# Victarry/Image-Generation-models

Hardware: AMD Instinct MI355X
Metric: ddpm_cifar10_32x32_train_images_per_sec (higher is better)
Workload: dtype bf16; 1 GPU; DDPM CIFAR-10 32x32, UNet 128/1-2-4, T=1000 (BASELINE configs[1]): train step B=128/GPU + hipGraph denoise step B=64; per_gpu_batch=128, global_batch=128, parallelism=dp1, step_launch=hipGraph replay, denoise_batch=64, rccl_ranks=1, state_finite=True, matmul=bf16 MFMA, fp32 accumulate

## Files before the change

image-generation-models_amd/csrc/conv_pw.hip:

```cpp
#include "tr_common.h"

#ifndef MI_PW_PABL
#define MI_PW_PABL 0
#endif
#ifndef MI_PW_GNSABL
#define MI_PW_GNSABL 0
#endif
#ifndef MI_PW_FXABL
#define MI_PW_FXABL 0
#endif
#ifdef MI_PW_TIMING
__device__ uint32_t g_pw_ts[1024 * 4 * 5 * 64];
__device__ __forceinline__ uint32_t pw_wlane(uint32_t val, uint32_t lane, uint32_t v) {
    uint32_t keep;
    asm volatile("s_mov_b32 %1, m0\n\ts_mov_b32 m0, %3\n\ts_nop 0\n\tv_writelane_b32 %0, %2, m0\n\ts_mov_b32 m0, %1"
                 : "+v"(v), "=&s"(keep) : "s"(__builtin_amdgcn_readfirstlane(val)), "s"(__builtin_amdgcn_readfirstlane(lane)));
    return v;
}
extern "C" int mi_debug_pw_ts(uint32_t* host_out) { return (int)hipMemcpyFromSymbol(host_out, HIP_SYMBOL(g_pw_ts), sizeof(g_pw_ts)); }
#endif

namespace {

typedef uint32_t u32x2 __attribute__((ext_vector_type(2)));
// ... 1 lines not shown
__device__ __attribute__((aligned(16))) uint32_t g_zero_page3[64];

struct PwArgs {
    const uint16_t* x; const uint16_t* x2; const uint16_t* w; const float* bias; const float* res; void* y;
    int N, H, W, K, Nc, K1, ldx, ldx2, ldy, ldr, accumulate, flip;
    int TH, TI, XP, tiles_per_img, xmap;
    int qmap, gx, gy;
    uint32_t tpi_magic, cpq_magic, nch_magic, cpg_magic; int ppx, cpq, lnsub;
    const void* zero;
    float* gsum;
    const float* coef;
    const float* sums; const float* gamma; const float* beta; const float* temb;
    int ldt, cpg, hw, ng; float eps;
    double icnt;
    int ksplit; float* sk_part; int* sk_flag;
};

constexpr int pw_xp(int pt) { return pt == 256 ? 320 : pt == 128 ? 192 : 128; }

__device__ __forceinline__ int pw_fastdiv(int x, uint32_t magic) { return magic ? (int)__umulhi((uint32_t)x, magic) : x; }
inline uint32_t pw_magic(int d) { return d > 1 ? (uint32_t)((0x100000000ULL + (unsigned)d - 1) / (unsigned)d) : 0u; }

__device__ __forceinline__ void glds16s(const void* sbase, uint32_t voff, uint32_t lds_dst) {
    const uint64_t p = (uint64_t)(uintptr_t)sbase;
    const uint32_t lo = __builtin_amdgcn_readfirstlane((uint32_t)p), hi = __builtin_amdgcn_readfirstlane((uint32_t)(p >> 32));
    const uint64_t q = ((uint64_t)hi << 32) | lo;
    const uint32_t dst = __builtin_amdgcn_readfirstlane(lds_dst);
    uint32_t keep;
    asm volatile("s_mov_b32 %0, m0\n\ts_mov_b32 m0, %3\n\ts_nop 0\n\tglobal_load_lds_dwordx4 %1, %2\n\ts_mov_b32 m0, %0"
                 : "=&s"(keep) : "v"(voff), "s"(q), "s"(dst) : "memory");
// ... 51 lines not shown
    constexpr bool TIMED = VAR == 0 && !IN32 && !F32;
    uint32_t tv[5] = {0u, 0u, 0u, 0u, 0u};
    uint64_t tprev = 0;
    if constexpr (TIMED) {
        tprev = __builtin_amdgcn_s_memtime();
        tv[4] = pw_wlane((uint32_t)wall_clock64(), 7, tv[4]);
        tv[4] = pw_wlane((uint32_t)tprev, 3, tv[4]);
    }
#define MI_PW_STAMP(SET, LANE) do { if constexpr (TIMED) { tv[SET] = pw_wlane((uint32_t)tprev, (LANE), tv[SET]); tprev = __builtin_amdgcn_s_memtime(); } } while (0)
#define MI_PW_NOW(LANE) do { if constexpr (TIMED) { tv[4] = pw_wlane((uint32_t)__builtin_amdgcn_s_memtime(), (LANE), tv[4]); } } while (0)
#else
#define MI_PW_STAMP(SET, LANE) do {} while (0)
#define MI_PW_NOW(LANE) do {} while (0)
#endif
    static_assert(PT != 256 || (VAR < 2 && !IN32 && !F32), "256-pixel tiles: the plain bf16 conv (with or without the GroupNorm sums)");
    constexpr bool FUSE = VAR >= 2, GNS = VAR == 1;
    static_assert(!F32 || (VAR == 0 && !IN32 && !OUT16), "exact-fp32 mode: the plain conv, fp32 in and out");
    constexpr int PCK = F32 ? 32 : 64;
    constexpr int ESZ = F32 ? 4 : 2, EPP = 16 / ESZ;
    constexpr int BH = PT / 32;
    constexpr int PXBUF = pw_xp(PT) * 128;
    constexpr int PXPW = pw_xp(PT) / 8 / 4;
    extern __shared__ __attribute__((aligned(16))) uint8_t lds_raw[];
    const uint32_t lds0 = (uint32_t)(uintptr_t)lds_raw;
    const int t = threadIdx.x, l = t & 63;
    const int wv = __builtin_amdgcn_readfirstlane(t >> 6);
    int bx = blockIdx.x;
    if (a.xmap) {
        const int xcd = bx & 7, slot = bx >> 3, q = pw_fastdiv(slot, a.tpi_magic);
        bx = (xcd + 8 * q) * a.tiles_per_img + (slot - q * a.tiles_per_img);
    }
// ... 29 lines not shown
        constexpr int ks0 = decltype(ksc)::value, over = ks0 >= 4 ? 1 : 0, ks = ks0 - 4 * over, part = decltype(partc)::value;
        constexpr int t0 = (9 * part + NPART - 1) / NPART, t1 = (9 * (part + 1) + NPART - 1) / NPART;
        const uint32_t voff = wl16 + (uint32_t)cof(ch + over) * 4096;
        static_for<t0, t1>([&](auto tc) {
            constexpr int tp = decltype(tc)::value;
            gload16s<ks * 1024>(WB[ks & 1][tp], wtap[tp], voff);
        });
    };

    auto load_w1 = [&](int ch, auto ksc, auto tapc) {
        constexpr int ks0 = decltype(ksc)::value, over = ks0 >= 4 ? 1 : 0, ks = ks0 - 4 * over, tp = decltype(tapc)::value;
        const uint32_t voff = wl16 + (uint32_t)cof(ch + over) * 4096;
        gload16s<ks * 1024>(WB[ks & 1][tp], wtap[tp], voff);
    };

    constexpr bool EARLYW = VAR < 2 && !IN32;
    if constexpr (EARLYW) {
        MI_PW_NOW(10);
        static_for<0, NPART>([&](auto pc) { load_w3(0, std::integral_constant<int, 0>{}, pc); });
        __builtin_amdgcn_sched_barrier(0);
    }


    int xpix[PXPW];
    const bool w8 = a.W == 8;
    const int xcol = ((l & 7) ^ (w8 ? (((l >> 4) & 3) | (((wv >> 1) & 1) << 2)) : ((4 * wv + (l >> 4)) & 7))) * EPP;
    int img0;
    {
        int y0;
        if (a.TI > 1) { img0 = bx * a.TI; y0 = 0; }
        else { img0 = pw_fastdiv(bx, a.tpi_magic); y0 = (bx - img0 * a.tiles_per_img) * a.TH; }
// ... 650 lines not shown
        __builtin_amdgcn_s_barrier();
        asm volatile("" ::: "memory");
        if (t < 32) {
            const int q = t >> 2, k = t & 3;
            const float v = red[(0 * 8 + q) * 4 + k] + red[(1 * 8 + q) * 4 + k] + red[(2 * 8 + q) * 4 + k] + red[(3 * 8 + q) * 4 + k];
            const int slab = (n0 >> 4) + q;
            if (slab * 16 < a.Nc) {
                const int img = a.TI > 1 ? img0 + (k >> 1) : img0;
                gsum_add(a.gsum, ((size_t)img * (a.Nc >> 4) + slab) * 2 + (k & 1), v);
            }
        }
        };
    __builtin_amdgcn_s_barrier();
    asm volatile("" ::: "memory");
    MI_PW_NOW(13);
    const bool tile16 = OUT16 && !a.res && !a.accumulate;
    if (tile16) {
        if constexpr (OUT16) {
            typedef __attribute__((address_space(3))) u32x2 lds_u32x2;
            typedef __attribute__((address_space(3))) u32x4 lds_u32x4e;
            if (live) {
#pragma unroll
                for (int rq = 0; rq < 4; ++rq) {
                    const int ck = 8 * wv + 2 * rq + (l >> 5);
                    typedef __attribute__((address_space(3))) f32x4 lds_f32x4b;
                    const f32x4 bq = *(lds_f32x4b*)(uintptr_t)(lds0 + BIASL + 16 * ck);
#pragma unroll
                    for (int i = 0; i < BH; ++i) {
                        const int p = ep_p0 + i * a.W;
                        *(lds_u32x2*)(uintptr_t)(lds0 + p * 256 + ((ck ^ ((p & 15) << 1)) << 3)) =
                            u32x2{pack_bf16(acc[i][4 * rq] + bq.x, acc[i][4 * rq + 1] + bq.y), pack_bf16(acc[i][4 * rq + 2] + bq.z, acc[i][4 * rq + 3] + bq.w)};
                    }
                }
            }
            __syncthreads();
            MI_PW_NOW(14);
            const int j = t & 15, col = n0 + 8 * j;
            float gs[2][2] = {{0.f, 0.f}, {0.f, 0.f}};
            if (col < a.Nc) {
#pragma unroll
                for (int it = 0; it < PT / 16; ++it) {
                    const int p = it * 16 + (t >> 4);
                    const u32x4 o = *(lds_u32x4e*)(uintptr_t)(lds0 + p * 256 + (((2 * j) ^ ((p & 15) << 1)) << 3));
                    *reinterpret_cast<u32x4*>(reinterpret_cast<uint16_t*>(a.y) + ((size_t)m0 + p) * a.ldy + col) = o;
                    if constexpr (GNS && MI_PW_GNSABL != 2) {
#pragma unroll
                        for (int q = 0; q < 4; ++q) {
                            const float e0 = __uint_as_float(o[q] << 16), e1 = __uint_as_float(o[q] & 0xffff0000u);
                            gs[PT >= 256 ? 0 : it >> 2][0] += e0 + e1; gs[PT >= 256 ? 0 : it >> 2][1] += e0 * e0 + e1 * e1;
                        }
                    }
// ... 820 lines not shown
        if (d->K % 128 || d->K1 % 128 || d->K1 <= 0 || d->K1 > d->K || d->Nc % 64 || d->ldx % 4 || (d->K1 != d->K && d->ldx2 % 4)) return false;
        return ((long)d->N * d->OH * d->OW) % 128 == 0;
    }
    if (f32) {
        if (d->KH != 1 || d->KW != 1 || d->pad != 0 || d->stride != 1 || d->mode != 0 || d->IH != d->OH || d->IW != d->OW) return false;
        if (d->K % 64 || d->K1 % 64 || d->K1 <= 0 || d->K1 > d->K || d->Nc % 64 || d->ldx % 4 || (d->K1 != d->K && d->ldx2 % 4)) return false;
        return ((long)d->N * d->OH * d->OW) % 128 == 0;
    }
    if (d->KH != 1 || d->KW != 1 || d->pad != 0 || d->stride != 1 || d->mode != 1) return false;
    if (d->IH != d->OH || d->IW != d->OW) return false;
    if (d->K % 128 || d->K1 % 128 || d->K1 <= 0 || d->K1 > d->K || d->Nc % 64 || d->ldx % 8 || (d->K1 != d->K && d->ldx2 % 8)) return false;
    return ((long)d->N * d->OH * d->OW) % 128 == 0;
}

struct PwGn { const float* sums; const float* gamma; const float* beta; const float* temb; int ldt, G; float eps; };

static int pw_launch(const char* who, const MiConvDesc* d, const void* x, const void* x2, const void* w_frag_bf16, const float* bias,
                     const float* residual, void* y, int out_bf16, int var, float* gsum, const float* coef, void* stream,
                     const PwGn* gn = nullptr, bool in32 = false, bool f32 = false) {
    PwArgs a{};
    if (!d || !x || !w_frag_bf16 || !y) return mi_set_error(-1, "%s: null argument", who);
    const int pt = pw_pick_tile(d, var, &a.TH, &a.TI, in32, f32, &a.ksplit);
    if (!pt) return mi_set_error(-1, "%s: descriptor not supported by the private-weight-stream conv kernel", who);
    int dev_ = 0;
    (void)hipGetDevice(&dev_);
    if (a.ksplit > 1) {
        uint8_t* ws = reinterpret_cast<uint8_t*>(g_pw_sk_ws[dev_ & 63].load(std::memory_order_acquire));
        a.sk_flag = reinterpret_cast<int*>(ws); a.sk_part = reinterpret_cast<float*>(ws + PW_SK_FLAG_BYTES);
#ifdef MI_PW_SK_ABL
        a.sk_flag = nullptr;
#endif
    }
    if (d->K1 != d->K && !x2) return mi_set_error(-1, "%s: two-source split without x2", who);
    if ((((uintptr_t)x | (uintptr_t)(x2 ? x2 : x) | (uintptr_t)w_frag_bf16) & 15) != 0) return mi_set_error(-1, "%s: operands must be 16-byte aligned", who);
    if (d->ldy % 8 || (residual && d->ldr % 4)) return mi_set_error(-1, "%s: output pixel stride must be a multiple of 8, the residual's of 4", who);
    if (var >= 2 && (a.TI != 1 || d->K1 != d->K))
        return mi_set_error(-1, "%s: the fused variants need one image per tile and one source", who);
    if (var == 2 && (!coef || ((uintptr_t)coef & 15)))
        return mi_set_error(-1, "%s: the fused variant needs a 16-byte aligned coefficient tensor", who);
    if (var == 3) {
        if (!gn || !gn->sums || !gn->gamma || !gn->beta || gn->G <= 0 || d->K % gn->G || (d->K / gn->G) % 16 || d->K / gn->G > 64)
            return mi_set_error(-1, "%s: sums, gamma, beta; K / G in {16, 32, 64}", who);
        if ((((uintptr_t)gn->gamma | (uintptr_t)gn->beta | (uintptr_t)gn->sums) & 7) || ((uintptr_t)gn->sums & 15) || (gn->temb && (((uintptr_t)gn->temb & 15) || gn->ldt % 4)))
            return mi_set_error(-1, "%s: misaligned GroupNorm operands", who);
        a.sums = gn->sums; a.gamma = gn->gamma; a.beta = gn->beta; a.temb = gn->temb; a.ldt = gn->ldt; a.cpg = d->K / gn->G;
        a.cpg_magic = pw_magic(a.cpg); a.ng = gn->G; a.hw = d->OH * d->OW; a.eps = gn->eps; a.icnt = 1.0 / (MI_GSUM_SCALE * (double)a.hw * (double)a.cpg);
    }
    if (var == 1 && (!gsum || d->Nc % 16)) return mi_set_error(-1, "%s: GroupNorm sums need Nc %% 16 == 0 and a sum buffer", who);
    a.x = (const uint16_t*)x; a.x2 = (const uint16_t*)(x2 ? x2 : x); a.w = (const uint16_t*)w_frag_bf16; a.bias = bias; a.res = residual; a.y = y;
    a.N = d->N; a.H = d->OH; a.W = d->OW; a.K = d->K; a.Nc = d->Nc; a.K1 = d->K1; a.ldx = d->ldx; a.ldx2 = x2 ? d->ldx2 : d->ldx;
    a.ldy = d->ldy; a.ldr = d->ldr; a.accumulate = d->accumulate; a.flip = d->transposed ? 1 : 0;
    a.gsum = gsum; a.coef = coef;
    a.tiles_per_img = a.TI > 1 ? 1 : a.H / a.TH;
    a.XP = a.TI * (a.TH + 2) * a.W;
    a.xmap = a.TI == 1 && a.tiles_per_img > 1 && a.N % 8 == 0;
    static std::atomic<const void*> zero_pages[64];
    const void* zero_page = zero_pages[dev_ & 63].load(std::memory_order_acquire);
    if (!zero_page) {
        void* p_ = nullptr;
        if (hipGetSymbolAddress(&p_, HIP_SYMBOL(g_zero_page3)) != hipSuccess || !p_) return mi_set_error(-1, "%s: zero page address", who);
        zero_pages[dev_ & 63].store(p_, std::memory_order_release);
        zero_page = p_;
    }
// ... 29 lines not shown
    } else if (in32) {
        if (pt == 64) switch (var) {
            case 1: if (out_bf16) MI_PW_GO_X(true, 1, 64); else MI_PW_GO_X(false, 1, 64); break;
            case 2: if (out_bf16) MI_PW_GO_X(true, 2, 64); else MI_PW_GO_X(false, 2, 64); break;
            case 3: if (out_bf16) MI_PW_GO_X(true, 3, 64); else MI_PW_GO_X(false, 3, 64); break;
            default: if (out_bf16) MI_PW_GO_X(true, 0, 64); else MI_PW_GO_X(false, 0, 64); break;
        } else switch (var) {
            case 1: if (out_bf16) MI_PW_GO_X(true, 1, 128); else MI_PW_GO_X(false, 1, 128); break;
            case 2: if (out_bf16) MI_PW_GO_X(true, 2, 128); else MI_PW_GO_X(false, 2, 128); break;
            case 3: if (out_bf16) MI_PW_GO_X(true, 3, 128); else MI_PW_GO_X(false, 3, 128); break;
            default: if (out_bf16) MI_PW_GO_X(true, 0, 128); else MI_PW_GO_X(false, 0, 128); break;
        }
    } else if (pt == 256) switch (var) {
        case 1: if (out_bf16) MI_PW_GO_T(true, 1, 256); else MI_PW_GO_T(false, 1, 256); break;
        default: if (out_bf16) MI_PW_GO_T(true, 0, 256); else MI_PW_GO_T(false, 0, 256); break;
    } else if (pt == 64) switch (var) {
        case 1: if (out_bf16) MI_PW_GO_T(true, 1, 64); else MI_PW_GO_T(false, 1, 64); break;
        case 2: if (out_bf16) MI_PW_GO_T(true, 2, 64); else MI_PW_GO_T(false, 2, 64); break;
        case 3: if (out_bf16) MI_PW_GO_T(true, 3, 64); else MI_PW_GO_T(false, 3, 64); break;
        default: if (out_bf16) MI_PW_GO_T(true, 0, 64); else MI_PW_GO_T(false, 0, 64); break;
    } else switch (var) {
        case 1: if (out_bf16) MI_PW_GO_T(true, 1, 128); else MI_PW_GO_T(false, 1, 128); break;
        case 2: if (out_bf16) MI_PW_GO_T(true, 2, 128); else MI_PW_GO_T(false, 2, 128); break;
        case 3: if (out_bf16) MI_PW_GO_T(true, 3, 128); else MI_PW_GO_T(false, 3, 128); break;
        default: if (out_bf16) MI_PW_GO_T(true, 0, 128); else MI_PW_GO_T(false, 0, 128); break;
    }
#undef MI_PW_GO_T
#undef MI_PW_GO_X
    hipError_t e_ = hipGetLastError();
    return e_ == hipSuccess ? 0 : mi_set_error((int)e_, "%s: %s", who, hipGetErrorString(e_));
// ... 43 lines not shown
    return (d && pw_pick_tile(d, 2, &th, &ti) && ti == 1 && d->K1 == d->K) ? 1 : 0;
}
extern "C" int mi_conv3x3_pw_gn_mish_tile(const MiConvDesc* d) {
    int th, ti;
    const int pt = d ? pw_pick_tile(d, 2, &th, &ti) : 0;
    return (pt && ti == 1 && d->K1 == d->K) ? pt : 0;
}

extern "C" int mi_conv3x3_pw(const MiConvDesc* d, const void* x, const void* x2, const void* w_frag_bf16, const float* bias,
                             const float* residual, void* y, int out_bf16, void* stream) {
    return pw_launch(__func__, d, x, x2, w_frag_bf16, bias, residual, y, out_bf16, 0, nullptr, nullptr, stream);
}
extern "C" int mi_conv3x3_pw_gnsums(const MiConvDesc* d, const void* x, const void* x2, const void* w_frag_bf16, const float* bias,
                                    const float* residual, void* y, int out_bf16, float* gsum, void* stream) {
    return pw_launch(__func__, d, x, x2, w_frag_bf16, bias, residual, y, out_bf16, 1, gsum, nullptr, stream);
}
extern "C" int mi_conv3x3_pw_x32_supported(const MiConvDesc* d) {
    int th, ti;
    return (d && pw_pick_tile(d, 0, &th, &ti, true)) ? 1 : 0;
}
extern "C" int mi_conv3x3_pw_x32_tile(const MiConvDesc* d) {
    int th, ti;
    return d ? pw_pick_tile(d, 0, &th, &ti, true) : 0;
}
extern "C" int mi_conv3x3_pw_x32(const MiConvDesc* d, const float* x, const float* x2, const void* w_frag_bf16, const float* bias,
                                 const float* residual, void* y, int out_bf16, float* gsum, void* stream) {
    return pw_launch(__func__, d, x, x2, w_frag_bf16, bias, residual, y, out_bf16, gsum ? 1 : 0, gsum, nullptr, stream, nullptr, true);
}
extern "C" int mi_conv3x3_pw_f32_tile(const MiConvDesc* d) {
    int th, ti;
// ... 341 lines not shown
```

image-generation-models_amd/src/models/ddpm.py:

```python
from __future__ import annotations

import math
import os
from functools import partial
from typing import Dict, List, Optional, Sequence, Tuple

import numpy as np
import torch
from torch import nn

from ..ops import functional as K
from .base import BaseModel, ValidationResult

_HEADS, _DHEAD = 4, 32
_GN_GROUPS = 8


def _mode_id(name: str) -> int:
    if name not in ("fp32", "bf16"):
        raise ValueError(f"compute mode must be 'fp32' or 'bf16', got {name!r}")
    return K.MODE_BF16 if name == "bf16" else K.MODE_FP32


class _Entry:
# ... 183 lines not shown
            raise ValueError("dim must be a multiple of 8")
        self.channels = channels
        self.dim = dim
        self.with_time_emb = bool(with_time_emb)
        arch = _Arch(dim, tuple(dim_mults), channels, out_dim, with_time_emb)
        object.__setattr__(self, "_arch", arch)
        self.compute_mode = os.environ.get("MI_DDPM_MODE", "fp32")
        self.block_storage = os.environ.get("MI_DDPM_STORAGE", "bf16")
        self.fuse_gn_conv = os.environ.get("MI_DDPM_FUSE_GN", "auto")
        self.s2_wgrad_tr = K.debug_knob("MI_DDPM_S2_TR", "1") != "0"
        self.final_block16 = K.debug_knob("MI_DDPM_FINAL16", "1") != "0"
        self.ends16 = K.debug_knob("MI_DDPM_ENDS16", "1") != "0"
        self.dual_out = K.debug_knob("MI_DDPM_DUAL_OUT", "1") != "0"
        self.fuse_ln_qkv = K.debug_knob("MI_DDPM_FUSE_LN", "1") != "0"
        self.fuse_ln_qkv_train = K.debug_knob("MI_DDPM_FUSE_LN_TRAIN", "1") != "0"
        self.small_cin_dual = K.debug_knob("MI_DDPM_CIN_DUAL", "1") != "0"
        self.cin_dual_chores = K.debug_knob("MI_DDPM_CIN_CHORES", "1") != "0"
        self.fold_attn = K.debug_knob("MI_DDPM_FOLD_ATTN", "0") == "1"
        self.small_cout_bwd1 = K.debug_knob("MI_DDPM_COUT_BWD1", "1") != "0"
        self.fuse_final = K.debug_knob("MI_DDPM_FUSE_FINAL", "1") != "0"
        self.accumulate_grads = False
        self.grad_ready_hook = None

        flat = torch.zeros(arch.flat_numel)
        for e in arch.entries:
            if e.init == "kaiming":
                w = torch.empty(e.shape)
                nn.init.kaiming_uniform_(w, a=math.sqrt(5))
                e.logical_view(flat).copy_(w)
            elif e.init == "ubias":
# ... 295 lines not shown
                ok2 = K.fast3x3_supported(B, inp.shape[1], inp.shape[2], co, co)
                lo16 = ok2[0] and ok2[1] and not (auto and K.conv3x3_uses_splitk(B, inp.shape[1], inp.shape[2], co, co))
            k1 = inp.shape[3] if x2 is not None else None
            c1_16 = (lo16 and ci % 32 == 0 and all(K.fast3x3_supported(B, inp.shape[1], inp.shape[2], ci, co, k1))
                     and not (auto and K.conv3x3_uses_splitk(B, inp.shape[1], inp.shape[2], ci, co, k1)))
            if (not c1_16 and lo16 and self.ends16 and x2 is None and K.small_cin_supported(3, ci, co, wgrad=True)
                    and K.small_cin_bf16_supported(3, B, inp.shape[1], inp.shape[2], ci, co, K.ld_of(inp))):
                c1_16 = True
            inp_c, x2_c = inp, x2
            if c1_16 and use_sh and inp.dtype == torch.float32 and inp.shape[3] % 8 == 0:
                inp_c, x2_c = shadow(inp), (shadow(x2) if x2 is not None else None)
            elif c1_16 and eval16 and x2 is None and id(inp) in sh:
                inp_c = sh[id(inp)][1]
            tb = tb_all[:, blk["tcol"]:blk["tcol"] + co] if tb_all is not None else None
            hw = inp.shape[1] * inp.shape[2]
            fmode = str(self.fuse_gn_conv)
            sums_ok = ((co // _GN_GROUPS) % 16 == 0 and hw % 32 == 0 and ci % 32 == 0
                       and all(K.fast3x3_supported(B, inp.shape[1], inp.shape[2], ci, co, k1)))
            fuse = (not record and mode == K.MODE_BF16 and fmode != "0" and c1_16 == lo16
                    and K.conv3x3_gn_mish_supported(B, inp.shape[1], inp.shape[2], co, co))
            if fuse and fmode == "auto":
                fuse = lo16 and sums_ok and K.conv3x3_pw_gn_mish_picked(B, inp.shape[1], inp.shape[2], co, co)
            sums = None
            if fuse and fmode in ("2", "auto") and sums_ok:
                sums = take_sums(co, inp.device)
            r_pre = None
            if (blk["res"] and x2 is None and sums is None and self.small_cin_dual and K.small_cin_supported(3, ci, co)
                    and K.small_cin_dual_supported(B, inp.shape[1], inp.shape[2], ci, co, K.ld_of(inp))):
                od = BF if (c1_16 and K.small_cin_bf16_supported(3, B, inp.shape[1], inp.shape[2], ci, co, K.ld_of(inp))) else torch.float32
                if not record and mode == K.MODE_BF16 and zpool[0] is None and str(self.fuse_gn_conv) != "0" and self.cin_dual_chores:
                    zpool[0] = torch.empty(2 * B * (sum(rb["cout"] // 16 + 1 for rb in A.res_blocks) + A.dim // 16 + 1), device=inp.device, dtype=torch.int64)
                    zfill = zpool[0]
                else:
                    zfill = None
                c1, r_pre = K.conv_small_cin_fwd_dual(inp, sv[pre + "block1.block.0.weight"], sv[pre + "block1.block.0.bias"],
                                                      sv[pre + "res_conv.weight"], sv[pre + "res_conv.bias"], co, out_dtype=od, zero=zfill,
                                                      gather=tb_pending.pop() if tb_pending else None)
            else:
                c1 = conv(inp_c, pre + "block1.block.0.", 3, 1, 1, x2=x2_c, out_dtype=BF if c1_16 else torch.float32, gn_sums=sums)
            c2 = None
            if fuse:
                if sums is not None:
                    st1 = None
                    c2 = K.conv3x3_gn_mish(c1, None, wf_sh[offs[pre + "block2.block.0.weight"]:], K=co, Nc=co, bias=sv[pre + "block2.block.0.bias"],
                                           gn=(sums, sv[pre + "block1.block.1.weight"], sv[pre + "block1.block.1.bias"], tb, _GN_GROUPS, 1e-5),
                                           wq=wfq_sh[offs[pre + "block2.block.0.weight"]:])
                else:
                    st1, coef = K.gn_stats_coef(c1, sv[pre + "block1.block.1.weight"], sv[pre + "block1.block.1.bias"], temb=tb)
                    c2 = K.conv3x3_gn_mish(c1, coef, wf_sh[offs[pre + "block2.block.0.weight"]:], K=co, Nc=co, bias=sv[pre + "block2.block.0.bias"],
                                           wq=wfq_sh[offs[pre + "block2.block.0.weight"]:])
                h1 = None
            if c2 is None:
                h1, st1 = K.gn_mish_fwd(c1, sv[pre + "block1.block.1.weight"], sv[pre + "block1.block.1.bias"], temb=tb,
                                        out_dtype=BF if lo16 else torch.float32)
                c2 = conv(h1, pre + "block2.block.0.", 3, 1, 1, out_dtype=BF if lo16 else torch.float32)
            r = inp
            if r_pre is not None:
                r = r_pre
            elif blk["res"]:
                r = None
                if inp_c is not inp and inp_c.dtype == BF and (x2 is None or x2_c is not None):
                    r = conv(inp_c, pre + "res_conv.", 1, x2=x2_c, soft=True)
                if r is None:
                    r = conv(inp, pre + "res_conv.", 1, x2=x2)
            if want_out16 and (use_sh or (eval16 and out16_in_eval)) and co % 32 == 0:
                out, st2, out16 = K.gn_mish_fwd(c2, sv[pre + "block2.block.1.weight"], sv[pre + "block2.block.1.bias"], residual=r, want16=True)
                sh[id(out)] = (out, out16)
            else:
                out, st2 = K.gn_mish_fwd(c2, sv[pre + "block2.block.1.weight"], sv[pre + "block2.block.1.bias"], residual=r)
            if record:
                tape.append(("res", blk, inp, x2, c1, st1, h1, c2, st2, out, inp_c, x2_c))
            return out

        def attention(at, inp, feeds_s2=False):
            pre = at["pre"]
            c = inp.shape[3]
            a16 = (mode == K.MODE_BF16 and self.block_storage in ("bf16", "auto") and B % 8 == 0
                   and all(K.fast1x1_supported(B, inp.shape[1], inp.shape[2], c, 3 * _HEADS * _DHEAD))
                   and all(K.fast1x1_supported(B, inp.shape[1], inp.shape[2], _HEADS * _DHEAD, c)))
            dt = BF if a16 else torch.float32
            nq = 3 * _HEADS * _DHEAD
            if (a16 and self.fuse_ln_qkv and (not record or self.fuse_ln_qkv_train) and inp.dtype == torch.float32
                    and K.ln_conv1x1_supported(B, inp.shape[1], inp.shape[2], c, nq, K.ld_of(inp))):
# ... 564 lines not shown
```

image-generation-models_amd/src/ops/functional.py:

```python
from __future__ import annotations

import ctypes as C
import functools
import os
from typing import Optional, Tuple

import torch

from .lib import ROWSUM_MAX, MiConvDesc, MiGnDesc, MiRowSum, MiWgradDesc, check, load_library

MODE_FP32, MODE_BF16 = 0, 1


def debug_knob(name: str, default: str) -> str:
    if os.environ.get("MI_DEBUG_KNOBS") == "1":
        return os.environ.get(name, default)
    return default
PROBE = None


CONV_AUTO = os.environ.get("MI_CONV_AUTO", "1") == "1"


USE_CONV_PW = CONV_AUTO and debug_knob("MI_CONV_PW", "1") == "1"
# ... 314 lines not shown
              "mi_conv3x3_bf16w_io")
    else:
        check(lib.mi_conv3x3_bf16w(C.byref(d), _p(x), _p(x2), _p(wsh), _p(bias), _p(residual), _p(out), _stream()),
              "mi_conv3x3_bf16w")
    if e0 is not None:
        bm, ck, sk = C.c_int(), C.c_int(), C.c_int()
        lib.mi_conv3x3_bf16w_tile(C.byref(d), io, C.byref(bm), C.byref(ck), C.byref(sk))
        nb = (N * H * W * K * _esz(x) + N * H * W * Nc * (_esz(out) * (2 if accumulate else 1) + _esz(residual))
              + ksize * ksize * K * Nc * 2)
        _probe_close(e0, f"conv3x3_halo_kernel<{bm.value}, {ck.value}, {ksize}, {'true' if sk.value else 'false'}, {io}, {8 if bm.value == 256 or (bm.value == 128 and ck.value == 64) else 4}>",
                     2.0 * N * H * W * Nc * K * ksize * ksize,
                     f"N{N} {H}x{W} K{K}{'(2src)' if x2 is not None else ''}->{Nc} flip{int(flip)} acc{int(accumulate)} io{io}", nb)
    return (out, y16) if want16 else out


def gn_stats_coef(x, gamma, beta, *, groups=8, eps=1e-5, temb=None):
    _need_gpu(x)
    N, H, W, Cc = x.shape
    stats = torch.empty((N, groups, 2), device=x.device, dtype=torch.float32)
    coef = torch.empty((3, N, Cc), device=x.device, dtype=torch.float32)
    d = MiGnDesc(N=N, HW=H * W, C=Cc, G=groups, eps=eps, ldx=ld_of(x), ldy=Cc, ldr=0)
    e0 = _probe_open()
    check(load_library().mi_gn_stats_coef(C.byref(d), _p(x), _p(gamma), _p(beta), _p(temb), ld_of(temb) if temb is not None else 0,
                                          _p(stats), _p(coef), _b16(x), _stream()), "mi_gn_stats_coef")
    if e0 is not None:
        _probe_close(e0, f"gn_mish_fwd_kernel<io{_b16(x)}> (statistics only)", 0.0, f"N{N} HW{H * W} C{Cc}", N * H * W * Cc * _esz(x))
    return stats, coef


GSUM_SCALE = float(1 << 20)
# ... 1409 lines not shown
```

image-generation-models_amd/src/ops/lib.py:

```python
from __future__ import annotations

import ctypes as C
import os

_PKG_ROOT = os.path.dirname(os.path.dirname(os.path.dirname(os.path.abspath(__file__))))
_LIB = None


def library_path() -> str:
    return os.environ.get("MI_DDPM_LIB", os.path.join(_PKG_ROOT, "lib", "libmi_ddpm.so"))


class MiConvDesc(C.Structure):
    _fields_ = [(n, C.c_int) for n in (
        "N", "IH", "IW", "OH", "OW", "K", "Nc", "KH", "KW", "stride", "pad", "transposed", "w_kn", "mode",
        "K1", "ldx", "ldx2", "ldy", "ldr", "accumulate")]


class MiWgradDesc(C.Structure):
    _fields_ = [(n, C.c_int) for n in (
        "N", "GH", "GW", "DH", "DW", "Ci", "Cj", "KH", "KW", "stride", "pad", "gather_i", "mode", "I1",
        "ldp", "ldp2", "ldq")]


# ... 78 lines not shown
    "mi_debug_conv_pw_splitk": [_I],
    "mi_ln_conv1x1_pw_supported": [C.POINTER(MiConvDesc)],
    "mi_ln_conv1x1_pw": [C.POINTER(MiConvDesc), _P, _P, _P, C.c_float, _P, _P, _P, _P],
    "mi_ln_conv1x1_pw_dual": [C.POINTER(MiConvDesc), _P, _P, _P, C.c_float, _P, _P, _P, _P, _I, _P],
    "mi_conv1x1_pw_f32_supported": [C.POINTER(MiConvDesc)],
    "mi_conv1x1_pw_f32": [C.POINTER(MiConvDesc), _P, _P, _P, _P, _P, _P, _P],
    "mi_pack_weights_f32frag": [_I, _P, _I, _P, _P, _P, _P],
    "mi_conv3x3_pw_x32_supported": [C.POINTER(MiConvDesc)],
    "mi_conv3x3_pw_x32_tile": [C.POINTER(MiConvDesc)],
    "mi_conv3x3_pw_x32": [C.POINTER(MiConvDesc), _P, _P, _P, _P, _P, _P, _I, _P, _P],
    "mi_conv3x3_pw": [C.POINTER(MiConvDesc), _P, _P, _P, _P, _P, _P, _I, _P],
    "mi_conv3x3_pw_gn_mish_supported": [C.POINTER(MiConvDesc)],
    "mi_conv1x1_pw_supported": [C.POINTER(MiConvDesc)],
    "mi_conv1x1_pw": [C.POINTER(MiConvDesc), _P, _P, _P, _P, _P, _P, _I, _P, _I, _P],
    "mi_conv3x3_pw_gnsums": [C.POINTER(MiConvDesc), _P, _P, _P, _P, _P, _P, _I, _P, _P],
    "mi_conv3x3_pw_gn_mish": [C.POINTER(MiConvDesc), _P, _P, _P, _P, _P, _I, _P],
    "mi_conv3x3_pw_gn_mish_sums": [C.POINTER(MiConvDesc), _P, _P, _P, _P, _P, _I, _I, _F, _P, _P, _P, _I, _P],
    "mi_conv3x3_pw_x32_gn_mish_supported": [C.POINTER(MiConvDesc)],
    "mi_conv3x3_pw_x32_gn_mish_tile": [C.POINTER(MiConvDesc)],
    "mi_conv3x3_pw_gn_mish_tile": [C.POINTER(MiConvDesc)],
    "mi_conv3x3_pw_x32_gn_mish": [C.POINTER(MiConvDesc), _P, _P, _P, _P, _P, _I, _P],
    "mi_conv3x3_pw_x32_gn_mish_sums": [C.POINTER(MiConvDesc), _P, _P, _P, _P, _P, _I, _I, _F, _P, _P, _P, _I, _P],
    "mi_gn_stats_coef": [C.POINTER(MiGnDesc), _P, _P, _P, _P, _I, _P, _P, _I, _P],
    "mi_conv3x3_gn_mish_supported": [C.POINTER(MiConvDesc)],
    "mi_conv3x3_gn_mish_tile": [C.POINTER(MiConvDesc), C.POINTER(C.c_int), C.POINTER(C.c_int)],
    "mi_conv3x3_gn_mish": [C.POINTER(MiConvDesc), _P, _P, _P, _P, _P, _I, _P],
    "mi_conv3x3_small_cin_fwd": [_I, _I, _I, _I, _I, _P, _I, _P, _P, _P, _I, _P],
    "mi_conv3x3_small_cin_wgrad": [_I, _I, _I, _I, _I, _P, _I, _P, _I, _P, _P],
    "mi_conv1x1_small_cout": [_I, _I, _I, _I, _P, _I, _P, _I, _P, _P, _P, _I, _I, _P],
    "mi_conv1x1_small_cout_ws": [_I, _I, _I, _I, _P, _I, _P, _I, _P, _P, _P, _I, _I, _P, _Z, _P],
# ... 150 lines not shown
```

include/mi_ddpm.h:

```cpp
#ifndef MI_DDPM_H
#define MI_DDPM_H
#include <stddef.h>
#include <stdint.h>

#ifdef __cplusplus
extern "C" {
#endif

#define MI_ABI_VERSION 4
#define MI_MODE_FP32 0
#define MI_MODE_BF16 1

int mi_abi_version(void);
const char* mi_last_error(void);

typedef struct MiConvDesc {
    int N;
    int IH, IW;
    int OH, OW;
    int K;
    int Nc;
    int KH, KW, stride, pad;
    int transposed;
    int w_kn;
// ... 63 lines not shown
int mi_ln_conv1x1_pw_dual(const MiConvDesc* d, const float* x, const float* ln_g, const float* ln_b, float eps, const void* w_frag_bf16,
                          const float* bias, void* y_bf16, void* ln_bf16, int ldl, void* stream);
int mi_conv1x1_pw_f32_supported(const MiConvDesc* d);
int mi_conv1x1_pw_f32(const MiConvDesc* d, const float* x, const float* x2, const float* w_frag_f32, const float* bias,
                      const float* residual, float* y, void* stream);
int mi_pack_weights_f32frag(int nent, const void* entries_dev, int total_tiles, const float* master, float* wdq32, float* wfq32,
                            void* stream);
int mi_debug_conv_pw_tile(int pt);
int mi_debug_conv_pw_auto256(int min_workgroups);
int mi_debug_conv1x1_pw_nloop(int on);
int mi_conv3x3_pw_tile(const MiConvDesc* d);
int mi_conv3x3_pw(const MiConvDesc* d, const void* x, const void* x2, const void* w_frag_bf16, const float* bias,
                  const float* residual, void* y, int out_bf16, void* stream);
int mi_conv3x3_pw_gnsums(const MiConvDesc* d, const void* x, const void* x2, const void* w_frag_bf16, const float* bias,
                         const float* residual, void* y, int out_bf16, float* gsum, void* stream);
int mi_conv3x3_pw_gn_mish_supported(const MiConvDesc* d);
int mi_conv3x3_pw_gn_mish_tile(const MiConvDesc* d);
int mi_conv3x3_pw_gn_mish(const MiConvDesc* d, const void* x, const float* coef, const void* w_frag_bf16, const float* bias,
                          void* y, int out_bf16, void* stream);
int mi_conv3x3_pw_gn_mish_sums(const MiConvDesc* d, const void* x, const float* sums, const float* gamma, const float* beta,
                               const float* temb, int ldt, int G, float eps, const void* w_frag_bf16, const float* bias,
                               void* y, int out_bf16, void* stream);
int mi_conv3x3_pw_x32_gn_mish_supported(const MiConvDesc* d);
int mi_conv3x3_pw_x32_gn_mish_tile(const MiConvDesc* d);
int mi_conv3x3_pw_x32_gn_mish(const MiConvDesc* d, const float* x, const float* coef, const void* w_frag_bf16, const float* bias,
                              void* y, int out_bf16, void* stream);
int mi_conv3x3_pw_x32_gn_mish_sums(const MiConvDesc* d, const float* x, const float* sums, const float* gamma, const float* beta,
                                   const float* temb, int ldt, int G, float eps, const void* w_frag_bf16, const float* bias,
                                   void* y, int out_bf16, void* stream);
int mi_conv1x1_pw_supported(const MiConvDesc* d);
// ... 296 lines not shown
```

Before: 26180 images/s.

## Fold GroupNorm+Mish into 3x3 conv epilogue for 8x8 resblocks

Adds conv kernel variants that compute GroupNorm statistics, the affine, Mish, the time-embedding add and optionally the residual add inside the conv epilogue, for 8x8 images where one tile covers whole images. The aim is to drop separate gn_mish_fwd launches and the extra re-reads of the conv output in the training forward pass. This costs more epilogue work and LDS reductions per tile, and it only applies to 8x8 layers, so the number of layers affected is small.

```diff
diff --git a/image-generation-models_amd/csrc/conv_pw.hip b/image-generation-models_amd/csrc/conv_pw.hip
--- a/image-generation-models_amd/csrc/conv_pw.hip
+++ b/image-generation-models_amd/csrc/conv_pw.hip
@@ -39,6 +39,7 @@
     int ldt, cpg, hw, ng; float eps;
     double icnt;
     int ksplit; float* sk_part; int* sk_flag;
+    void* y2; float* stats; const float* gres; uint16_t* y16; int ldy2, ldgr, ldy16;
 };
 
 constexpr int pw_xp(int pt) { return pt == 256 ? 320 : pt == 128 ? 192 : 128; }
@@ -120,7 +121,9 @@
 #define MI_PW_NOW(LANE) do {} while (0)
 #endif
     static_assert(PT != 256 || (VAR < 2 && !IN32 && !F32), "256-pixel tiles: the plain bf16 conv (with or without the GroupNorm sums)");
-    constexpr bool FUSE = VAR >= 2, GNS = VAR == 1;
+    constexpr bool FUSE = VAR == 2 || VAR == 3, GNS = VAR == 1;
+    constexpr bool GNF = VAR == 4 || VAR == 5;
+    static_assert(!GNF || (OUT16 && !IN32 && !F32 && (PT == 64 || PT == 128)), "GroupNorm fold: bf16 conv output, 64- or 128-pixel tiles");
     static_assert(!F32 || (VAR == 0 && !IN32 && !OUT16), "exact-fp32 mode: the plain conv, fp32 in and out");
     constexpr int PCK = F32 ? 32 : 64;
     constexpr int ESZ = F32 ? 4 : 2, EPP = 16 / ESZ;
@@ -180,7 +183,7 @@
         gload16s<ks * 1024>(WB[ks & 1][tp], wtap[tp], voff);
     };
 
-    constexpr bool EARLYW = VAR < 2 && !IN32;
+    constexpr bool EARLYW = (VAR < 2 || GNF) && !IN32;
     if constexpr (EARLYW) {
         MI_PW_NOW(10);
         static_for<0, NPART>([&](auto pc) { load_w3(0, std::integral_constant<int, 0>{}, pc); });
@@ -861,7 +864,7 @@
     __builtin_amdgcn_s_barrier();
     asm volatile("" ::: "memory");
     MI_PW_NOW(13);
-    const bool tile16 = OUT16 && !a.res && !a.accumulate;
+    const bool tile16 = GNF || (OUT16 && !a.res && !a.accumulate);
     if (tile16) {
         if constexpr (OUT16) {
             typedef __attribute__((address_space(3))) u32x2 lds_u32x2;
@@ -882,6 +885,122 @@
             }
             __syncthreads();
             MI_PW_NOW(14);
+            if constexpr (GNF) {
+                constexpr int NI = PT / 64, NR = PT / 16;
+                const int j = t & 15, pr = t >> 4, col = n0 + 8 * j;
+                const f32x4 gq0 = *reinterpret_cast<const f32x4*>(a.gamma + col), gq1 = *reinterpret_cast<const f32x4*>(a.gamma + col + 4);
+                const f32x4 bq0 = *reinterpret_cast<const f32x4*>(a.beta + col), bq1 = *reinterpret_cast<const f32x4*>(a.beta + col + 4);
+                f32x4 tq[NI][2];
+#pragma unroll
+                for (int im = 0; im < NI; ++im) {
+                    tq[im][0] = tq[im][1] = f32x4{0.f, 0.f, 0.f, 0.f};
+                    if (a.temb) {
+                        const float* tp = a.temb + (size_t)(img0 + im) * a.ldt + col;
+                        tq[im][0] = *reinterpret_cast<const f32x4*>(tp); tq[im][1] = *reinterpret_cast<const f32x4*>(tp + 4);
+                    }
+                }
+                f32x4 rq[VAR == 5 ? NR : 1][2];
+                if constexpr (VAR == 5) {
+#pragma unroll
+                    for (int it = 0; it < NR; ++it) {
+                        const float* rp = a.gres + ((size_t)m0 + it * 16 + pr) * a.ldgr + col;
+                        rq[it][0] = *reinterpret_cast<const f32x4*>(rp); rq[it][1] = *reinterpret_cast<const f32x4*>(rp + 4);
+                    }
+                }
+                u32x4 o[NR];
+#pragma unroll
+                for (int it = 0; it < NR; ++it) {
+                    const int p = it * 16 + pr;
+                    o[it] = *(lds_u32x4e*)(uintptr_t)(lds0 + p * 256 + (((2 * j) ^ ((p & 15) << 1)) << 3));
+                    *reinterpret_cast<u32x4*>(reinterpret_cast<uint16_t*>(a.y) + ((size_t)m0 + p) * a.ldy + col) = o[it];
+                }
+                auto gn_sum = [&](float (&v)[NI], float* red) {
+#pragma unroll
+                    for (int im = 0; im < NI; ++im) {
+                        v[im] += __shfl_xor(v[im], 1, 64);
+                        if (a.cpg >= 32) v[im] += __shfl_xor(v[im], 2, 64);
+                        if (a.cpg >= 64) v[im] += __shfl_xor(v[im], 4, 64);
+                        v[im] += __shfl_xor(v[im], 16, 64); v[im] += __shfl_xor(v[im], 32, 64);
+                    }
+                    if (l < 16) {
+#pragma unroll
+                        for (int im = 0; im < NI; ++im) red[(wv * 16 + l) * NI + im] = v[im];
+                    }
+                    asm volatile("s_waitcnt lgkmcnt(0)" ::: "memory");
+                    __builtin_amdgcn_s_barrier();
+                    asm volatile("" ::: "memory");
+#pragma unroll
+                    for (int im = 0; im < NI; ++im)
+                        v[im] = (red[(0 * 16 + j) * NI + im] + red[(1 * 16 + j) * NI + im]) + (red[(2 * 16 + j) * NI + im] + red[(3 * 16 + j) * NI + im]);
+                };
+                float* red = reinterpret_cast<float*>(lds_raw + PT * 512);
+                const float cnt = 64.f * (float)a.cpg;
+                float mean[NI], rstd[NI];
+#pragma unroll
+                for (int im = 0; im < NI; ++im) {
+                    mean[im] = 0.f;
+#pragma unroll
+                    for (int k = 0; k < 4; ++k)
+#pragma unroll
+                        for (int q = 0; q < 4; ++q) mean[im] += __uint_as_float(o[4 * im + k][q] << 16) + __uint_as_float(o[4 * im + k][q] & 0xffff0000u);
+                }
+                gn_sum(mean, red);
+#pragma unroll
+                for (int im = 0; im < NI; ++im) {
+                    mean[im] = mean[im] / cnt;
+                    rstd[im] = 0.f;
+#pragma unroll
+                    for (int k = 0; k < 4; ++k)
+#pragma unroll
+                        for (int q = 0; q < 4; ++q) {
+                            const float d0 = __uint_as_float(o[4 * im + k][q] << 16) - mean[im], d1 = __uint_as_float(o[4 * im + k][q] & 0xffff0000u) - mean[im];
+                            rstd[im] += d0 * d0; rstd[im] += d1 * d1;
+                        }
+                }
+                gn_sum(rstd, red + 128);
+#pragma unroll
+                for (int im = 0; im < NI; ++im) rstd[im] = 1.0f / sqrtf(rstd[im] / cnt + a.eps);
+                if (pr == 0 && ((8 * j) & (a.cpg - 1)) == 0) {
+                    const int g = col >> (31 - __builtin_clz(a.cpg));
+#pragma unroll
+                    for (int im = 0; im < NI; ++im)
+                        *reinterpret_cast<f32x2*>(a.stats + ((size_t)(img0 + im) * a.ng + g) * 2) = f32x2{mean[im], rstd[im]};
+                }
+#pragma unroll
+                for (int im = 0; im < NI; ++im) {
+                    float ga[8], be[8];
+#pragma unroll
+                    for (int e = 0; e < 8; ++e) {
+                        ga[e] = (e < 4 ? gq0[e] : gq1[e - 4]) * rstd[im];
+                        be[e] = (e < 4 ? bq0[e] : bq1[e - 4]) - mean[im] * ga[e];
+                    }
+#pragma unroll
+                    for (int k = 0; k < 4; ++k) {
+                        const int it = 4 * im + k;
+                        const size_t m = (size_t)m0 + it * 16 + pr;
+                        float hv[8];
+#pragma unroll
+                        for (int e = 0; e < 8; ++e) {
+                            const float xv = (e & 1) ? __uint_as_float(o[it][e >> 1] & 0xffff0000u) : __uint_as_float(o[it][e >> 1] << 16);
+                            hv[e] = mish_fast_f(xv * ga[e] + be[e]) + (e < 4 ? tq[im][0][e] : tq[im][1][e - 4]);
+                        }
+                        if constexpr (VAR == 4) {
+                            *reinterpret_cast<u32x4*>(reinterpret_cast<uint16_t*>(a.y2) + m * a.ldy2 + col) =
+                                u32x4{pack_bf16(hv[0], hv[1]), pack_bf16(hv[2], hv[3]), pack_bf16(hv[4], hv[5]), pack_bf16(hv[6], hv[7])};
+                        } else {
+#pragma unroll
+                            for (int e = 0; e < 8; ++e) hv[e] += e < 4 ? rq[it][0][e] : rq[it][1][e - 4];
+                            float* yp = reinterpret_cast<float*>(a.y2) + m * a.ldy2 + col;
+                            *reinterpret_cast<f32x4*>(yp) = f32x4{hv[0], hv[1], hv[2], hv[3]};
+                            *reinterpret_cast<f32x4*>(yp + 4) = f32x4{hv[4], hv[5], hv[6], hv[7]};
+                            if (a.y16)
+                                *reinterpret_cast<u32x4*>(a.y16 + m * a.ldy16 + col) =
+                                    u32x4{pack_bf16(hv[0], hv[1]), pack_bf16(hv[2], hv[3]), pack_bf16(hv[4], hv[5]), pack_bf16(hv[6], hv[7])};
+                        }
+                    }
+                }
+                return;
+            }
             const int j = t & 15, col = n0 + 8 * j;
             float gs[2][2] = {{0.f, 0.f}, {0.f, 0.f}};
             if (col < a.Nc) {
@@ -1732,12 +1851,22 @@
 }
 
 struct PwGn { const float* sums; const float* gamma; const float* beta; const float* temb; int ldt, G; float eps; };
+struct PwFold { void* out; int ldo; float* stats; const float* res; int ldr; void* out16; int ldo16; };
+bool pw_fold_ok(const MiConvDesc* d, int G, int pt, int TH, int TI) {
+    if (G <= 0 || d->Nc % G) return false;
+    const int cpg = d->Nc / G;
+    return (pt == 64 || pt == 128) && d->OH == 8 && d->OW == 8 && TH == d->OH && TI == pt / 64 && d->Nc % 128 == 0
+        && (cpg == 16 || cpg == 32 || cpg == 64) && !d->accumulate;
+}
 
 static int pw_launch(const char* who, const MiConvDesc* d, const void* x, const void* x2, const void* w_frag_bf16, const float* bias,
                      const float* residual, void* y, int out_bf16, int var, float* gsum, const float* coef, void* stream,
-                     const PwGn* gn = nullptr, bool in32 = false, bool f32 = false) {
+                     const PwGn* gn = nullptr, bool in32 = false, bool f32 = false, const PwFold* fold = nullptr) {
     PwArgs a{};
     if (!d || !x || !w_frag_bf16 || !y) return mi_set_error(-1, "%s: null argument", who);
+    const bool gnf = var >= 4;
+    const int lvar = var;
+    if (gnf) var = 0;
     const int pt = pw_pick_tile(d, var, &a.TH, &a.TI, in32, f32, &a.ksplit);
     if (!pt) return mi_set_error(-1, "%s: descriptor not supported by the private-weight-stream conv kernel", who);
     int dev_ = 0;
@@ -1765,6 +1894,18 @@
         a.cpg_magic = pw_magic(a.cpg); a.ng = gn->G; a.hw = d->OH * d->OW; a.eps = gn->eps; a.icnt = 1.0 / (MI_GSUM_SCALE * (double)a.hw * (double)a.cpg);
     }
     if (var == 1 && (!gsum || d->Nc % 16)) return mi_set_error(-1, "%s: GroupNorm sums need Nc %% 16 == 0 and a sum buffer", who);
+    if (gnf) {
+        if (!gn || !fold || !gn->gamma || !gn->beta || !fold->out || !fold->stats || in32 || f32 || !out_bf16 || residual || !pw_fold_ok(d, gn->G, pt, a.TH, a.TI))
+            return mi_set_error(-1, "%s: the GroupNorm fold needs 8x8 images, Nc %% 128 == 0, groups of 16 / 32 / 64 channels, a bf16 conv output without residual", who);
+        if (lvar == 5 && (!fold->res || fold->ldr % 4 || ((uintptr_t)fold->res & 15) || (fold->out16 && (fold->ldo16 % 8 || ((uintptr_t)fold->out16 & 15)))))
+            return mi_set_error(-1, "%s: the GroupNorm-2 fold needs a 16-byte aligned fp32 residual (stride %% 4) and bf16 copy (stride %% 8)", who);
+        if ((((uintptr_t)gn->gamma | (uintptr_t)gn->beta | (uintptr_t)fold->out | (uintptr_t)y) & 15) || ((uintptr_t)fold->stats & 7) || fold->ldo % (lvar == 4 ? 8 : 4)
+            || (gn->temb && (((uintptr_t)gn->temb & 15) || gn->ldt % 4)))
+            return mi_set_error(-1, "%s: misaligned GroupNorm operands", who);
+        a.gamma = gn->gamma; a.beta = gn->beta; a.temb = gn->temb; a.ldt = gn->ldt; a.cpg = d->Nc / gn->G; a.ng = gn->G; a.eps = gn->eps;
+        a.y2 = fold->out; a.ldy2 = fold->ldo; a.stats = fold->stats; a.gres = fold->res; a.ldgr = fold->ldr;
+        a.y16 = reinterpret_cast<uint16_t*>(fold->out16); a.ldy16 = fold->ldo16;
+    }
     a.x = (const uint16_t*)x; a.x2 = (const uint16_t*)(x2 ? x2 : x); a.w = (const uint16_t*)w_frag_bf16; a.bias = bias; a.res = residual; a.y = y;
     a.N = d->N; a.H = d->OH; a.W = d->OW; a.K = d->K; a.Nc = d->Nc; a.K1 = d->K1; a.ldx = d->ldx; a.ldx2 = x2 ? d->ldx2 : d->ldx;
     a.ldy = d->ldy; a.ldr = d->ldr; a.accumulate = d->accumulate; a.flip = d->transposed ? 1 : 0;
@@ -1824,6 +1965,9 @@
     } else if (pt == 256) switch (var) {
         case 1: if (out_bf16) MI_PW_GO_T(true, 1, 256); else MI_PW_GO_T(false, 1, 256); break;
         default: if (out_bf16) MI_PW_GO_T(true, 0, 256); else MI_PW_GO_T(false, 0, 256); break;
+    } else if (gnf) {
+        if (pt == 64) { if (lvar == 4) MI_PW_GO_T(true, 4, 64); else MI_PW_GO_T(true, 5, 64); }
+        else { if (lvar == 4) MI_PW_GO_T(true, 4, 128); else MI_PW_GO_T(true, 5, 128); }
     } else if (pt == 64) switch (var) {
         case 1: if (out_bf16) MI_PW_GO_T(true, 1, 64); else MI_PW_GO_T(false, 1, 64); break;
         case 2: if (out_bf16) MI_PW_GO_T(true, 2, 64); else MI_PW_GO_T(false, 2, 64); break;
@@ -1897,6 +2041,26 @@
 extern "C" int mi_conv3x3_pw_gnsums(const MiConvDesc* d, const void* x, const void* x2, const void* w_frag_bf16, const float* bias,
                                     const float* residual, void* y, int out_bf16, float* gsum, void* stream) {
     return pw_launch(__func__, d, x, x2, w_frag_bf16, bias, residual, y, out_bf16, 1, gsum, nullptr, stream);
+}
+extern "C" int mi_conv3x3_pw_gn_fold_supported(const MiConvDesc* d, int groups) {
+    int th, ti, ks = 1;
+    if (!d || d->mode != 1) return 0;
+    const int pt = pw_pick_tile(d, 0, &th, &ti, false, false, &ks);
+    return (pt && pw_fold_ok(d, groups, pt, th, ti)) ? 1 : 0;
+}
+extern "C" int mi_conv3x3_pw_gn1_fold(const MiConvDesc* d, const void* x, const void* x2, const void* w_frag_bf16, const float* bias, void* c,
+                                      const float* gamma, const float* beta, const float* temb, int ldt, int groups, float eps, float* stats,
+                                      void* h, int ldh, void* stream) {
+    const PwGn gn{nullptr, gamma, beta, temb, ldt, groups, eps};
+    const PwFold fo{h, ldh, stats, nullptr, 0, nullptr, 0};
+    return pw_launch(__func__, d, x, x2, w_frag_bf16, bias, nullptr, c, 1, 4, nullptr, nullptr, stream, &gn, false, false, &fo);
+}
+extern "C" int mi_conv3x3_pw_gn2_fold(const MiConvDesc* d, const void* x, const void* x2, const void* w_frag_bf16, const float* bias, void* c,
+                                      const float* gamma, const float* beta, const float* temb, int ldt, int groups, float eps, float* stats,
+                                      const float* res, int ldr, float* out, int ldo, void* out16, int ldo16, void* stream) {
+    const PwGn gn{nullptr, gamma, beta, temb, ldt, groups, eps};
+    const PwFold fo{out, ldo, stats, res, ldr, out16, ldo16};
+    return pw_launch(__func__, d, x, x2, w_frag_bf16, bias, nullptr, c, 1, 5, nullptr, nullptr, stream, &gn, false, false, &fo);
 }
 extern "C" int mi_conv3x3_pw_x32_supported(const MiConvDesc* d) {
     int th, ti;
diff --git a/image-generation-models_amd/src/models/ddpm.py b/image-generation-models_amd/src/models/ddpm.py
--- a/image-generation-models_amd/src/models/ddpm.py
+++ b/image-generation-models_amd/src/models/ddpm.py
@@ -221,6 +221,7 @@
         self.dual_out = K.debug_knob("MI_DDPM_DUAL_OUT", "1") != "0"
         self.fuse_ln_qkv = K.debug_knob("MI_DDPM_FUSE_LN", "1") != "0"
         self.fuse_ln_qkv_train = K.debug_knob("MI_DDPM_FUSE_LN_TRAIN", "1") != "0"
+        self.fold_gn_tile = True
         self.small_cin_dual = K.debug_knob("MI_DDPM_CIN_DUAL", "1") != "0"
         self.cin_dual_chores = K.debug_knob("MI_DDPM_CIN_CHORES", "1") != "0"
         self.fold_attn = K.debug_knob("MI_DDPM_FOLD_ATTN", "0") == "1"
@@ -546,6 +547,7 @@
                 inp_c = sh[id(inp)][1]
             tb = tb_all[:, blk["tcol"]:blk["tcol"] + co] if tb_all is not None else None
             hw = inp.shape[1] * inp.shape[2]
+            fold, h1, st1 = False, None, None
             fmode = str(self.fuse_gn_conv)
             sums_ok = ((co // _GN_GROUPS) % 16 == 0 and hw % 32 == 0 and ci % 32 == 0
                        and all(K.fast3x3_supported(B, inp.shape[1], inp.shape[2], ci, co, k1)))
@@ -569,7 +571,17 @@
                                                       sv[pre + "res_conv.weight"], sv[pre + "res_conv.bias"], co, out_dtype=od, zero=zfill,
                                                       gather=tb_pending.pop() if tb_pending else None)
             else:
-                c1 = conv(inp_c, pre + "block1.block.0.", 3, 1, 1, x2=x2_c, out_dtype=BF if c1_16 else torch.float32, gn_sums=sums)
+                fold = (record and self.fold_gn_tile and mode == K.MODE_BF16 and lo16 and c1_16 and hw == 64 and inp_c.dtype == BF
+                        and (x2 is None or (x2_c is not None and x2_c.dtype == BF)))
+                f1 = None
+                if fold:
+                    f1 = K.conv3x3_gn_fold(inp_c, wfq_sh[offs[pre + "block1.block.0.weight"]:], sv[pre + "block1.block.1.weight"],
+                                           sv[pre + "block1.block.1.bias"], K=ci, Nc=co, x2=x2_c, bias=sv[pre + "block1.block.0.bias"],
+                                           temb=tb, groups=_GN_GROUPS)
+                if f1 is not None:
+                    c1, st1, h1 = f1
+                else:
+                    c1 = conv(inp_c, pre + "block1.block.0.", 3, 1, 1, x2=x2_c, out_dtype=BF if c1_16 else torch.float32, gn_sums=sums)
             c2 = None
             if fuse:
                 if sums is not None:
@@ -582,23 +594,41 @@
                     c2 = K.conv3x3_gn_mish(c1, coef, wf_sh[offs[pre + "block2.block.0.weight"]:], K=co, Nc=co, bias=sv[pre + "block2.block.0.bias"],
                                            wq=wfq_sh[offs[pre + "block2.block.0.weight"]:])
                 h1 = None
+            def res_input():
+                r = inp
+                if r_pre is not None:
+                    r = r_pre
+                elif blk["res"]:
+                    r = None
+                    if inp_c is not inp and inp_c.dtype == BF and (x2 is None or x2_c is not None):
+                        r = conv(inp_c, pre + "res_conv.", 1, x2=x2_c, soft=True)
+                    if r is None:
+                        r = conv(inp, pre + "res_conv.", 1, x2=x2)
+                return r
+
+            out16_now = want_out16 and (use_sh or (eval16 and out16_in_eval)) and co % 32 == 0
+            r = out = None
             if c2 is None:
-                h1, st1 = K.gn_mish_fwd(c1, sv[pre + "block1.block.1.weight"], sv[pre + "block1.block.1.bias"], temb=tb,
-                                        out_dtype=BF if lo16 else torch.float32)
-                c2 = conv(h1, pre + "block2.block.0.", 3, 1, 1, out_dtype=BF if lo16 else torch.float32)
-            r = inp
-            if r_pre is not None:
-                r = r_pre
-            elif blk["res"]:
-                r = None
-                if inp_c is not inp and inp_c.dtype == BF and (x2 is None or x2_c is not None):
-                    r = conv(inp_c, pre + "res_conv.", 1, x2=x2_c, soft=True)
-                if r is None:
-                    r = conv(inp, pre + "res_conv.", 1, x2=x2)
-            if want_out16 and (use_sh or (eval16 and out16_in_eval)) and co % 32 == 0:
+                if h1 is None:
+                    h1, st1 = K.gn_mish_fwd(c1, sv[pre + "block1.block.1.weight"], sv[pre + "block1.block.1.bias"], temb=tb,
+                                            out_dtype=BF if lo16 else torch.float32)
+                if fold and h1.dtype == BF:
+                    r = res_input()
+                    f2 = K.conv3x3_gn_fold(h1, wfq_sh[offs[pre + "block2.block.0.weight"]:], sv[pre + "block2.block.1.weight"],
+                                           sv[pre + "block2.block.1.bias"], K=co, Nc=co, bias=sv[pre + "block2.block.0.bias"],
+                                           groups=_GN_GROUPS, residual=r, want16=out16_now)
+                    if f2 is not None:
+                        c2, st2, out = f2[:3]
+                        if out16_now:
+                            sh[id(out)] = (out, f2[3])
+                if c2 is None:
+                    c2 = conv(h1, pre + "block2.block.0.", 3, 1, 1, out_dtype=BF if lo16 else torch.float32)
+            if r is None:
+                r = res_input()
+            if out is None and out16_now:
                 out, st2, out16 = K.gn_mish_fwd(c2, sv[pre + "block2.block.1.weight"], sv[pre + "block2.block.1.bias"], residual=r, want16=True)
                 sh[id(out)] = (out, out16)
-            else:
+            elif out is None:
                 out, st2 = K.gn_mish_fwd(c2, sv[pre + "block2.block.1.weight"], sv[pre + "block2.block.1.bias"], residual=r)
             if record:
                 tape.append(("res", blk, inp, x2, c1, st1, h1, c2, st2, out, inp_c, x2_c))
diff --git a/image-generation-models_amd/src/ops/functional.py b/image-generation-models_amd/src/ops/functional.py
--- a/image-generation-models_amd/src/ops/functional.py
+++ b/image-generation-models_amd/src/ops/functional.py
@@ -352,6 +352,45 @@
     return (out, y16) if want16 else out
 
 
+def conv3x3_gn_fold(x, wq, gamma, beta, *, K, Nc, x2=None, bias=None, flip=False, groups=8, eps=1e-5, temb=None, residual=None, want16=False):
+    _need_gpu(x)
+    N, H, W, K1 = x.shape
+    if x2 is None:
+        K1 = K
+    if not (USE_CONV_PW and wq is not None and _b16(x) and (x2 is None or _b16(x2)) and H == 8 and W == 8 and Nc % groups == 0):
+        return None
+    d = MiConvDesc(N=N, IH=H, IW=W, OH=H, OW=W, K=K, Nc=Nc, KH=3, KW=3, stride=1, pad=1, transposed=int(flip), w_kn=0, mode=MODE_BF16,
+                   K1=K1, ldx=ld_of(x), ldx2=ld_of(x2) if x2 is not None else 0, ldy=Nc, ldr=0, accumulate=0)
+    if not (_pick_pw(N, H, W, K, Nc, d) and _query("mi_conv3x3_pw_gn_fold_supported", d, groups)):
+        return None
+    if residual is not None and (residual.dtype != torch.float32 or ld_of(residual) % 4 or residual.data_ptr() % 16):
+        return None
+    if temb is not None and (ld_of(temb) % 4 or temb.data_ptr() % 16):
+        return None
+    lib = load_library()
+    c = new_act(N, H, W, Nc, x, torch.bfloat16)
+    stats = torch.empty((N, groups, 2), device=x.device, dtype=torch.float32)
+    ldt = ld_of(temb) if temb is not None else 0
+    e0 = _probe_open()
+    if residual is None:
+        h = new_act(N, H, W, Nc, x, torch.bfloat16)
+        check(lib.mi_conv3x3_pw_gn1_fold(C.byref(d), _p(x), _p(x2), _p(wq), _p(bias), _p(c), _p(gamma), _p(beta), _p(temb), ldt, groups, eps,
+                                         _p(stats), _p(h), ld_of(h), _stream()), "mi_conv3x3_pw_gn1_fold")
+        ret, var, extra = (c, stats, h), 4, 2
+    else:
+        out = new_act(N, H, W, Nc, x, torch.float32)
+        out16 = new_act(N, H, W, Nc, x, torch.bfloat16) if want16 else None
+        check(lib.mi_conv3x3_pw_gn2_fold(C.byref(d), _p(x), _p(x2), _p(wq), _p(bias), _p(c), _p(gamma), _p(beta), _p(temb), ldt, groups, eps,
+                                         _p(stats), _p(residual), ld_of(residual), _p(out), ld_of(out), _p(out16),
+                                         ld_of(out16) if want16 else 0, _stream()), "mi_conv3x3_pw_gn2_fold")
+        ret, var, extra = ((c, stats, out, out16) if want16 else (c, stats, out)), 5, 8 + (2 if want16 else 0)
+    if e0 is not None:
+        nb = N * H * W * K * 2 + N * H * W * Nc * (2 + extra) + 9 * K * Nc * 2
+        _probe_close(e0, _pw_sym(d, True).replace(", 0, 0, ", f", {var}, 0, "), 2.0 * N * H * W * Nc * K * 9,
+                     f"N{N} {H}x{W} K{K}{'(2src)' if x2 is not None else ''}->{Nc} + GroupNorm {var - 3} + Mish", nb)
+    return ret
+
+
 def gn_stats_coef(x, gamma, beta, *, groups=8, eps=1e-5, temb=None):
     _need_gpu(x)
     N, H, W, Cc = x.shape
diff --git a/image-generation-models_amd/src/ops/lib.py b/image-generation-models_amd/src/ops/lib.py
--- a/image-generation-models_amd/src/ops/lib.py
+++ b/image-generation-models_amd/src/ops/lib.py
@@ -116,6 +116,9 @@
     "mi_conv1x1_pw_supported": [C.POINTER(MiConvDesc)],
     "mi_conv1x1_pw": [C.POINTER(MiConvDesc), _P, _P, _P, _P, _P, _P, _I, _P, _I, _P],
     "mi_conv3x3_pw_gnsums": [C.POINTER(MiConvDesc), _P, _P, _P, _P, _P, _P, _I, _P, _P],
+    "mi_conv3x3_pw_gn_fold_supported": [C.POINTER(MiConvDesc), _I],
+    "mi_conv3x3_pw_gn1_fold": [C.POINTER(MiConvDesc), _P, _P, _P, _P, _P, _P, _P, _P, _I, _I, _F, _P, _P, _I, _P],
+    "mi_conv3x3_pw_gn2_fold": [C.POINTER(MiConvDesc), _P, _P, _P, _P, _P, _P, _P, _P, _I, _I, _F, _P, _P, _I, _P, _I, _P, _I, _P],
     "mi_conv3x3_pw_gn_mish": [C.POINTER(MiConvDesc), _P, _P, _P, _P, _P, _I, _P],
     "mi_conv3x3_pw_gn_mish_sums": [C.POINTER(MiConvDesc), _P, _P, _P, _P, _P, _I, _I, _F, _P, _P, _P, _I, _P],
     "mi_conv3x3_pw_x32_gn_mish_supported": [C.POINTER(MiConvDesc)],
diff --git a/include/mi_ddpm.h b/include/mi_ddpm.h
--- a/include/mi_ddpm.h
+++ b/include/mi_ddpm.h
@@ -101,6 +101,13 @@
                   const float* residual, void* y, int out_bf16, void* stream);
 int mi_conv3x3_pw_gnsums(const MiConvDesc* d, const void* x, const void* x2, const void* w_frag_bf16, const float* bias,
                          const float* residual, void* y, int out_bf16, float* gsum, void* stream);
+int mi_conv3x3_pw_gn_fold_supported(const MiConvDesc* d, int groups);
+int mi_conv3x3_pw_gn1_fold(const MiConvDesc* d, const void* x, const void* x2, const void* w_frag_bf16, const float* bias, void* c,
+                           const float* gamma, const float* beta, const float* temb, int ldt, int groups, float eps, float* stats,
+                           void* h, int ldh, void* stream);
+int mi_conv3x3_pw_gn2_fold(const MiConvDesc* d, const void* x, const void* x2, const void* w_frag_bf16, const float* bias, void* c,
+                           const float* gamma, const float* beta, const float* temb, int ldt, int groups, float eps, float* stats,
+                           const float* res, int ldr, float* out, int ldo, void* out16, int ldo16, void* stream);
 int mi_conv3x3_pw_gn_mish_supported(const MiConvDesc* d);
 int mi_conv3x3_pw_gn_mish_tile(const MiConvDesc* d);
 int mi_conv3x3_pw_gn_mish(const MiConvDesc* d, const void* x, const float* coef, const void* w_frag_bf16, const float* bias,
```

After: 26440 images/s (median of 6 runs). Within noise of the previous version (+1.0%).
